# lhn0323/BEVFUSION-3D_object_detection

Hardware: AMD Instinct MI355X
Metric: nuScenes frames/sec (6-cam+LiDAR BEVFusion fwd+bwd) (higher is better)
Workload: dtype bf16; 1 GPU; full: BEVFusion camera+LiDAR (ResNet-50, LSS 6x256x704, hard voxelize 40k pts, sparse encoder, ConvFuser, SECOND/SECONDFPN, TransFusion head + Hungarian targets + focal/L1/gaussian-focal losses) fwd + bwd + clip + AdamW, bf16 autocast, fp32 index paths; global_batch=4, points_per_frame=40000, parallelism=independent frames per rank, execution=eager launches on 2 HIP queues (camera / BEV chain, LiDAR branch), view_transform_conv_dtype=bf16, head_fp32_conv=three bf16 products per multiply, fp32 accumulation (2^-16 relative per product), dense_weight_gradients=one grouped launch per tile shape at the end of the backward pass, backward_pass_thread=caller, trainable_params=37361053

## Files before the change

bevfusion-3d_object_detection_amd/_lib.py:

```python
import ctypes
import os

import torch

_HERE = os.path.dirname(os.path.abspath(__file__))
LIB_PATH = os.path.join(_HERE, "csrc", "libbevfusion_hip.so")

_c_int = ctypes.c_int
_c_vp = ctypes.c_void_p
_c_sz = ctypes.c_size_t

SIGNATURES = {
    "bfhip_abi_version": (_c_int, []),
    "bfhip_last_error": (ctypes.c_char_p, []),
    "bfhip_profile_enable": (None, [_c_int]),
    "bfhip_profile_read": (_c_int, [_c_int, _c_vp, _c_vp, _c_int]),
    "bfhip_bev_pool_fwd": (_c_int, [_c_vp] * 5 + [_c_int] * 7 + [_c_vp, _c_vp]),
    "bfhip_bev_pool_bwd": (_c_int, [_c_vp] * 5 + [_c_int] * 8 + [_c_vp, _c_vp]),
    "bfhip_dynamic_voxelize": (_c_int, [_c_vp, _c_vp, _c_int, _c_int, _c_vp, _c_vp, _c_vp]),
    "bfhip_hard_voxelize_workspace_bytes": (_c_sz, [_c_int, _c_int, _c_int]),
    "bfhip_hard_voxelize": (_c_int, [_c_vp, _c_int, _c_int, _c_vp, _c_vp, _c_vp, _c_vp, _c_vp,
                                     _c_int, _c_int, _c_vp, _c_sz, _c_vp, _c_vp]),
    "bfhip_bev_plan_workspace_bytes": (_c_sz, [ctypes.c_longlong, ctypes.c_longlong]),
    "bfhip_bev_plan": (_c_int, [_c_vp] * 7 + [_c_int] * 4 + [_c_vp] * 3 + [_c_vp] * 11 + [_c_int, _c_vp, _c_sz, _c_vp]),
# ... 93 lines not shown
                                     [_c_vp] * 4 + [_c_vp, _c_int, _c_vp, _c_vp, _c_vp]),
    "bfhip_bn2d_bwd_mask": (_c_int, [_c_vp] * 5 + [ctypes.c_longlong, _c_int, _c_int] + [_c_vp] * 4 + [_c_vp, _c_sz, _c_vp]),
    "bfhip_adamw_segment_bytes": (_c_int, []),
    "bfhip_adamw_chunk_elems": (_c_int, []),
    "bfhip_adamw_step": (_c_int, [_c_vp, _c_vp, _c_vp, _c_int, _c_vp, _c_vp] + [ctypes.c_float] * 6 + [_c_vp]),
    "bfhip_adamw_step_groups": (_c_int, [_c_vp, _c_vp, _c_vp, _c_int, _c_vp, _c_vp, _c_vp, _c_vp, _c_int, ctypes.c_float, _c_vp]),
    "bfhip_query_losses": (_c_int, [_c_vp] * 7 + [_c_int] * 6 + [ctypes.c_float, ctypes.c_float] + [_c_vp] * 4),
    "bfhip_swin_attn_supported": (_c_int, [_c_int] * 7),
    "bfhip_swin_attn_parts": (_c_int, [_c_int] * 4),
    "bfhip_swin_attn_fwd": (_c_int, [_c_vp, ctypes.c_longlong, _c_vp] + [_c_int] * 5 + [ctypes.c_float, _c_vp, _c_vp, _c_vp]),
    "bfhip_swin_attn_bwd": (_c_int, [_c_vp, ctypes.c_longlong, _c_vp, _c_vp, _c_vp, _c_vp] + [_c_int] * 5 +
                            [ctypes.c_float, _c_vp, _c_vp, _c_int, _c_vp]),
    "bfhip_layernorm_supported": (_c_int, [ctypes.c_longlong, _c_int, _c_int, _c_int]),
    "bfhip_layernorm_parts": (_c_int, [ctypes.c_longlong, _c_int]),
    "bfhip_layernorm_fwd": (_c_int, [_c_vp, _c_vp, _c_vp, ctypes.c_longlong, _c_vp, _c_vp, ctypes.c_longlong, _c_int, ctypes.c_float] +
                            [_c_int] * 3 + [_c_vp] * 4),
    "bfhip_layernorm_bwd": (_c_int, [_c_vp] * 6 + [ctypes.c_longlong, ctypes.c_longlong] + [_c_int] * 4 + [_c_vp] * 3 + [_c_int] +
                            [_c_vp] * 3),
    "bfhip_bn_eval_supported": (_c_int, [ctypes.c_longlong, _c_int, _c_int]),
    "bfhip_bn_eval_parts": (_c_int, [ctypes.c_longlong, _c_int, _c_int]),
    "bfhip_bn_eval_fwd": (_c_int, [_c_vp] * 6 + [ctypes.c_longlong, _c_int, _c_int, ctypes.c_float, _c_int, _c_vp, _c_vp]),
    "bfhip_bn_eval_bwd": (_c_int, [_c_vp] * 6 + [ctypes.c_longlong, _c_int, _c_int, ctypes.c_float, _c_int] + [_c_vp] * 5),
    "bfhip_img_preprocess_max_samples": (_c_int, []),
    "bfhip_img_preprocess": (_c_int, [_c_vp] + [_c_int] * 5 + [_c_vp, _c_vp, ctypes.c_float, _c_int, _c_int, _c_int, _c_int,
                                      _c_vp, _c_vp]),
    "bfhip_image_aug_max_taps": (_c_int, []),
    "bfhip_image_aug_max_cams": (_c_int, []),
    "bfhip_image_aug_supported": (_c_int, [_c_int] * 8),
    "bfhip_image_aug": (_c_int, [_c_vp, _c_int, _c_int, _c_vp, _c_vp, ctypes.c_longlong, _c_int, _c_int, _c_vp, _c_int, _c_int,
                                 _c_vp, _c_vp, ctypes.c_float] + [_c_int] * 4 + [_c_vp, _c_vp]),
    "bfhip_image_aug_masked": (_c_int, [_c_vp, _c_vp, _c_int, _c_int, _c_vp, _c_vp, ctypes.c_longlong, _c_int, _c_int, _c_vp, _c_int,
                                        _c_int, _c_vp, _c_vp, ctypes.c_float] + [_c_int] * 4 + [_c_vp, _c_vp]),
    "bfhip_points_aug_block": (_c_int, []),
    "bfhip_points_aug_workspace_bytes": (_c_sz, [ctypes.c_longlong, _c_int]),
    "bfhip_points_aug": (_c_int, [_c_vp, _c_int, _c_int, _c_vp, _c_vp, _c_vp, _c_sz, _c_vp]),
    "bfhip_points_aug_max_boxes": (_c_int, []),
    "bfhip_points_aug_paste": (_c_int, [_c_vp, _c_vp, _c_int, _c_int, _c_vp, _c_vp, _c_vp, _c_sz, _c_vp]),
    "bfhip_points_aug_max_sweeps": (_c_int, []),
    "bfhip_points_aug_sweeps": (_c_int, [_c_vp, _c_vp, _c_vp, _c_int, _c_int, _c_vp, _c_vp, _c_vp, _c_sz, _c_vp]),
    "bfhip_query_init_supported": (_c_int, [_c_int] * 8),
    "bfhip_query_init_workspace_bytes": (_c_sz, [_c_int] * 4),
    "bfhip_query_init_fwd": (_c_int, [_c_vp] + [ctypes.c_longlong] * 4 + [_c_int] * 4 + [ctypes.c_uint, _c_vp, ctypes.c_longlong,
                                      ctypes.c_longlong] + [_c_int] * 4 + [_c_vp] * 6 + [_c_sz, _c_vp]),
    "bfhip_query_init_bwd": (_c_int, [_c_vp, _c_vp, _c_int, _c_int, _c_int, ctypes.c_longlong, _c_int, _c_vp, _c_vp]),
    "bfhip_jpeg_parse": (_c_int, [_c_vp, _c_sz, _c_vp]),
    "bfhip_jpeg_entropy_decode": (_c_int, [_c_vp, _c_sz, _c_vp, _c_vp, _c_sz]),
    "bfhip_jpeg_decode": (_c_int, [_c_vp, _c_vp, _c_int, _c_vp, _c_sz, _c_vp, _c_sz, _c_vp, _c_sz, _c_vp]),
    "bfhip_points_in_boxes_block": (_c_int, []),
    "bfhip_points_in_boxes_max_boxes": (_c_int, []),
    "bfhip_points_in_boxes_workspace_bytes": (_c_sz, [ctypes.c_longlong, _c_int]),
    "bfhip_points_in_boxes_count": (_c_int, [_c_vp, ctypes.c_longlong, _c_int, _c_vp, _c_int, _c_vp, _c_vp, _c_vp, _c_sz, _c_vp]),
    "bfhip_points_in_boxes_gather": (_c_int, [_c_vp, ctypes.c_longlong, _c_int, _c_vp, _c_int, _c_vp, _c_vp, ctypes.c_longlong,
                                              _c_vp, ctypes.c_longlong, _c_vp, _c_sz, _c_vp]),
}


class ImgDesc(ctypes.Structure):
    _fields_ = [("data", _c_vp), ("h", _c_int), ("w", _c_int)]

_lib = None


def load():
    global _lib
    if _lib is None:
        if not os.path.exists(LIB_PATH):
            raise RuntimeError(
                "libbevfusion_hip.so not found at %s: build it with "
                "`python -c 'import __graft_entry__ as g; g.build()'` (hipcc, gfx950). "
                "There is no CPU fallback." % LIB_PATH)
        lib = ctypes.CDLL(LIB_PATH)
        for name, (res, args) in SIGNATURES.items():
            fn = getattr(lib, name)
            fn.restype = res
            fn.argtypes = args
        _lib = lib
    return _lib


_torch_ext = False


def torch_ext():
    global _torch_ext
    if _torch_ext is False:
        _torch_ext = None
        path = os.path.join(_HERE, "csrc", "bfhip_torch_ext.so")
        if os.environ.get("BFHIP_TORCH_EXT", "1") == "1" and os.path.exists(path):
            import importlib.util
            load()
            try:
                spec = importlib.util.spec_from_file_location("bfhip_torch_ext", path)
                mod = importlib.util.module_from_spec(spec)
                spec.loader.exec_module(mod)
                if mod.abi_version() == load().bfhip_abi_version():
                    _torch_ext = mod
            except (ImportError, OSError) as e:
                import warnings
                warnings.warn("bfhip_torch_ext not usable (%s); using the ctypes binding" % e)
    return _torch_ext


def check(rc, what):
    if rc != 0:
        msg = load().bfhip_last_error().decode("utf-8", "replace")
        raise RuntimeError("%s failed (rc=%d): %s" % (what, rc, msg))
# ... 64 lines not shown
```

bevfusion-3d_object_detection_amd/csrc/torch_binding.cpp:

```cpp
#include <torch/extension.h>
#include <torch/csrc/autograd/engine.h>
#include <torch/csrc/autograd/graph_task.h>
#include <c10/hip/HIPStream.h>
#include <c10/hip/HIPGuard.h>
#include <ATen/hip/impl/HIPStreamMasqueradingAsCUDA.h>
#include <hip/hip_runtime_api.h>

#include <map>
#include <mutex>
#include <vector>

#include "../../include/bevfusion_hip.h"

namespace {

using torch::Tensor;
using torch::autograd::AutogradContext;
using torch::autograd::tensor_list;

inline void *cur_stream(const Tensor &t) { return (void *)c10::hip::getCurrentHIPStream(t.get_device()).stream(); }
inline int dt_code(const Tensor &t) { return t.scalar_type() == at::kBFloat16 ? 1 : 0; }
inline void check(int rc, const char *what) {
  TORCH_CHECK(rc == 0, what, " failed (rc=", rc, "): ", bfhip_last_error());
}
// ... 403 lines not shown
    }
    dy = as_nhwc_bf16(dy);
    if (ctx->needs_input_grad(0)) {
      if (dgrad_lib) out[0] = add_grad(lib_dgrad(dy, x, weight, stride, pad, dil), d_alias, fork);
      else out[0] = hip_dgrad(dy, x, weight, wt, stride, pad, dil, d_alias, fork == 2 ? 2 : 1);
    }
    if (ctx->needs_input_grad(1)) out[1] = launch_wgrad(x, dy, weight, stride, pad, dil);
    if (has_bias && ctx->needs_input_grad(2)) out[2] = bias_grad(dy).to((at::ScalarType)g[6]);
    return out;
  }
};

tensor_list conv2d(const Tensor &x, const Tensor &weight, const c10::optional<Tensor> &bias, int64_t stride, int64_t pad, int64_t dil,
                   bool emit_stats, bool dgrad_lib, int64_t fork, const c10::optional<Tensor> &wt) {
  return ConvFn::apply(x, weight, bias, stride, pad, dil, emit_stats, dgrad_lib, fork, wt);
}

class LibConvFn : public torch::autograd::Function<LibConvFn> {
 public:
  static Tensor forward(AutogradContext *ctx, const Tensor &x_, const Tensor &weight, int64_t stride, int64_t pad, int64_t dil,
                        bool dgrad_hip, const c10::optional<Tensor> &wt) {
    Tensor x = as_nhwc_bf16(x_);
    Tensor w = weight.scalar_type() == at::kBFloat16 ? weight : weight.to(at::kBFloat16);
    Tensor y;
    {
      c10::impl::ExcludeDispatchKeyGuard no_autocast(c10::DispatchKey::AutocastCUDA);
      y = at::conv2d(x, w, {}, {stride, stride}, {pad, pad}, {dil, dil});
    }
    ctx->save_for_backward({x, weight, (wt.has_value() && wt->defined()) ? *wt : Tensor()});
    ctx->saved_data["geom"] = std::vector<int64_t>{stride, pad, dil, dgrad_hip ? 1 : 0};
    return y;
  }

  static tensor_list backward(AutogradContext *ctx, tensor_list grads) {
    auto saved = ctx->get_saved_variables();
    const Tensor &x = saved[0], &weight = saved[1], &wt = saved[2];
    const auto g = ctx->saved_data["geom"].toIntVector();
    const int64_t stride = g[0], pad = g[1], dil = g[2];
    tensor_list out(7);
    if (!grads[0].defined()) return out;
    Tensor dy = as_nhwc_bf16(grads[0]);
    if (ctx->needs_input_grad(0))
      out[0] = g[3] ? hip_dgrad(dy, x, weight, wt, stride, pad, dil, Tensor(), 1) : lib_dgrad(dy, x, weight, stride, pad, dil);
    if (ctx->needs_input_grad(1)) out[1] = launch_wgrad(x, dy, weight, stride, pad, dil);
    return out;
  }
};

Tensor lib_conv2d(const Tensor &x, const Tensor &weight, int64_t stride, int64_t pad, int64_t dil, bool dgrad_hip,
                  const c10::optional<Tensor> &wt) {
  return LibConvFn::apply(x, weight, stride, pad, dil, dgrad_hip, wt);
}

}

PYBIND11_MODULE(TORCH_EXTENSION_NAME, m) {
  m.doc() = "C++ autograd front-ends over libbevfusion_hip.so (include/bevfusion_hip.h)";
  m.def("bn2d", &bn2d, "fused BatchNorm2d(+residual)(+ReLU), channels-last, training mode; optional statistics partials of the producing conv",
        pybind11::arg("x"), pybind11::arg("residual"), pybind11::arg("weight"), pybind11::arg("bias"), pybind11::arg("running_mean"),
        pybind11::arg("running_var"), pybind11::arg("eps"), pybind11::arg("momentum"), pybind11::arg("relu"),
        pybind11::arg("partial") = c10::optional<Tensor>(), pybind11::arg("relu_bits") = false);
  m.def("bn1d", &bn1d, "fused BatchNorm1d(+residual)(+ReLU) on f32[N, C], training mode");
  m.def("conv2d", &conv2d, "dense convolution on csrc/conv2d.hip (conv2d.py::_Conv2dFunction): [y, partial (empty without statistics)[, x']]",
        pybind11::arg("x"), pybind11::arg("weight"), pybind11::arg("bias"), pybind11::arg("stride"), pybind11::arg("pad"), pybind11::arg("dil"),
        pybind11::arg("emit_stats"), pybind11::arg("dgrad_lib"), pybind11::arg("fork"), pybind11::arg("wt"));
  m.def("lib_conv2d", &lib_conv2d, "library forward, HIP weight gradient (conv2d.py::_LibConvHipWgradFunction)", pybind11::arg("x"),
        pybind11::arg("weight"), pybind11::arg("stride"), pybind11::arg("pad"), pybind11::arg("dil"), pybind11::arg("dgrad_hip"), pybind11::arg("wt"));
  m.def("defer_wgrad", &defer_wgrad, "queue a layer's weight gradient for the grouped launch at the end of the running backward pass");
  m.def("set_wgrad_grouped", [](bool on) { g_grouped = on; });
  m.def("pending_wgrads", &pending_wgrads);
  m.def("abi_version", []() { return bfhip_abi_version(); });
}
```

bevfusion-3d_object_detection_amd/depth_lss.py:

```python
import os
from typing import Tuple

import torch
from torch import nn

from . import _lib
from .bn2d import bn_act
from .conv2d import Conv2d
from .ops import bev_pool
from .registry import MODELS


BF16_BEV_OUT = os.environ.get("BFHIP_LIFT_SPLAT_BF16_OUT", "1") == "1"
CAMERA_MAJOR = os.environ.get("BFHIP_LIFT_SPLAT_ORDER", "0") == "1"
BF16_FEAT = os.environ.get("BFHIP_LIFT_SPLAT_BF16_FEAT", "1") == "1"


def _inverse(m):
    return torch.linalg.inv_ex(m, check_errors=False).inverse


def gen_dx_bx(xbound, ybound, zbound):
    rows = [xbound, ybound, zbound]
    dx = torch.Tensor([row[2] for row in rows])
    bx = torch.Tensor([row[0] + row[2] / 2.0 for row in rows])
    nx = torch.LongTensor([int((row[1] - row[0]) / row[2]) for row in rows])
    return dx, bx, nx


class BevPlan:

    def __init__(self, B, N, D, HW, nx, device, with_reference_outputs=False, with_geometry=False):
        self.B, self.N, self.D, self.HW = B, N, D, HW
        self.nx = [int(v) for v in nx]
        self.nprime = B * N * D * HW
        self.out_cells = B * self.nx[2] * self.nx[0] * self.nx[1]
        self.mmax = min(self.nprime, self.out_cells)
        i32 = dict(dtype=torch.int32, device=device)
        self.sorted_pd = torch.empty(self.nprime, **i32)
        self.starts = torch.empty(self.mmax, **i32)
        self.lengths = torch.empty(self.mmax, **i32)
        self.cell_of_interval = torch.empty(self.mmax, **i32)
        self.interval_order = torch.empty(self.mmax, **i32) if CAMERA_MAJOR else None
        self.counts = torch.zeros(2, **i32)
        self.cell_of_point = torch.empty(self.nprime, **i32)
        self.geom_sorted = torch.empty((self.nprime, 4), **i32) if with_reference_outputs else None
        self.ranks_sorted = torch.empty(self.nprime, dtype=torch.int64, device=device) if with_reference_outputs else None
        self.kept = torch.empty(self.nprime, dtype=torch.uint8, device=device) if with_reference_outputs else None
        self.geom_xyz = torch.empty((self.nprime, 3), dtype=torch.float32, device=device) if with_geometry else None
        nbytes = _lib.load().bfhip_bev_plan_workspace_bytes(self.nprime, self.out_cells)
        self.workspace = torch.empty(nbytes, dtype=torch.uint8, device=device)

    def build(self, frustum, post_trans, post_rots_inv, combine, c2l_trans, extra_rots, extra_trans, origin, dx):
        f32 = lambda t: t.contiguous().float()
        args = [f32(frustum), f32(post_trans), f32(post_rots_inv), f32(combine), f32(c2l_trans), f32(extra_rots),
                f32(extra_trans)]
        import ctypes
        nx_host = (ctypes.c_int32 * 3)(*self.nx)
        with torch.cuda.device(self.sorted_pd.device):
            rc = _lib.load().bfhip_bev_plan(
                *[_lib.ptr(a) for a in args], self.B, self.N, self.D, self.HW, _lib.host_f32(origin), _lib.host_f32(dx),
                nx_host, _lib.ptr(self.sorted_pd), _lib.ptr(self.starts), _lib.ptr(self.lengths),
                _lib.ptr(self.cell_of_interval), _lib.ptr(self.interval_order), _lib.ptr(self.counts), _lib.ptr(self.cell_of_point),
                _lib.ptr(self.geom_sorted), _lib.ptr(self.ranks_sorted), _lib.ptr(self.kept), _lib.ptr(self.geom_xyz),
                self.mmax, _lib.ptr(self.workspace), self.workspace.numel(), _lib.stream_of(self.sorted_pd))
        _lib.check(rc, "bev_plan")
        self._keepalive = args
        return self
# ... 7 lines not shown
        assert depth.dtype == torch.float32 and feat.dtype in (torch.float32, torch.bfloat16)
        f16 = 1 if feat.dtype == torch.bfloat16 else 0
        P, C = feat.shape
        assert P == plan.B * plan.N * plan.HW and depth.shape == (P, plan.D)
        assert out_dtype in (torch.float32, torch.bfloat16)
        out = torch.empty((plan.B, plan.nx[2], plan.nx[0], plan.nx[1], C), dtype=out_dtype, device=feat.device)
        with torch.cuda.device(feat.device):
            rc = _lib.load().bfhip_lift_splat_fwd(
                _lib.ptr(depth), depth.stride(0), _lib.ptr(feat), f16, feat.stride(0), _lib.ptr(plan.sorted_pd),
                _lib.ptr(plan.starts), _lib.ptr(plan.lengths), _lib.ptr(plan.cell_of_interval), _lib.ptr(plan.interval_order),
                _lib.ptr(plan.counts), plan.mmax, C, plan.out_cells, _lib.ptr(out), 1 if out_dtype == torch.bfloat16 else 0,
                _lib.stream_of(feat))
        _lib.check(rc, "lift_splat_fwd")
        ctx.save_for_backward(depth, feat)
        ctx.plan = plan
        return out

    @staticmethod
    def backward(ctx, out_grad):
        depth, feat = ctx.saved_tensors
        plan = ctx.plan
        out_grad = out_grad.contiguous()
        if out_grad.dtype not in (torch.float32, torch.bfloat16):
            out_grad = out_grad.float()
        P, C = feat.shape
        d_depth = torch.empty((P, plan.D), dtype=torch.float32, device=feat.device)
        d_feat = torch.empty((P, C), dtype=feat.dtype, device=feat.device)
        with torch.cuda.device(feat.device):
            rc = _lib.load().bfhip_lift_splat_bwd(
                _lib.ptr(out_grad), 1 if out_grad.dtype == torch.bfloat16 else 0, _lib.ptr(depth), depth.stride(0), _lib.ptr(feat),
                1 if feat.dtype == torch.bfloat16 else 0, feat.stride(0),
                _lib.ptr(plan.cell_of_point), plan.B * plan.N, plan.D, plan.HW, C, _lib.ptr(d_depth), plan.D,
                _lib.ptr(d_feat), C, _lib.stream_of(feat))
        _lib.check(rc, "lift_splat_bwd")
        return d_depth, d_feat, None, None


class _SplitDepthFeat(torch.autograd.Function):

    @staticmethod
    def forward(ctx, x, D, C):
        ctx.shape, ctx.D, ctx.C = x.shape, D, C
        return x[:, :D].float(), x[:, D:D + C].contiguous()

    @staticmethod
    def backward(ctx, g_logits, g_feat):
        D, C = ctx.D, ctx.C
        dx = torch.empty(ctx.shape, dtype=torch.bfloat16, device=g_logits.device)
        dx[:, :D].copy_(g_logits)
        dx[:, D:D + C].copy_(g_feat)
        if ctx.shape[1] > D + C:
            dx[:, D + C:].zero_()
        return dx, None, None


def lift_splat(depth, feat, plan, out_dtype=torch.float32):
    return _LiftSplat.apply(depth, feat, plan, out_dtype)


class BaseViewTransform(nn.Module):

    def __init__(self, in_channels: int, out_channels: int, image_size: Tuple[int, int],
                 feature_size: Tuple[int, int], xbound, ybound, zbound, dbound) -> None:
        super().__init__()
        self.in_channels = in_channels
        self.image_size = image_size
        self.feature_size = feature_size
        self.xbound, self.ybound, self.zbound, self.dbound = xbound, ybound, zbound, dbound
        dx, bx, nx = gen_dx_bx(xbound, ybound, zbound)
        self.dx = nn.Parameter(dx, requires_grad=False)
        self.bx = nn.Parameter(bx, requires_grad=False)
        self.nx = nn.Parameter(nx, requires_grad=False)
        self.C = out_channels
        self.conv_dtype = None
        self.frustum = self.create_frustum()
        self.D = self.frustum.shape[0]
        self.fp16_enabled = False
        self._nx_host = [int(v) for v in nx]
        self._dx_host = [float(v) for v in dx]
        self._origin_host = [float(v) for v in (bx - dx / 2.0)]

    def create_frustum(self):
        iH, iW = self.image_size
        fH, fW = self.feature_size
        ds = torch.arange(*self.dbound, dtype=torch.float).view(-1, 1, 1).expand(-1, fH, fW)
        D = ds.shape[0]
        xs = torch.linspace(0, iW - 1, fW, dtype=torch.float).view(1, 1, fW).expand(D, fH, fW)
        ys = torch.linspace(0, iH - 1, fH, dtype=torch.float).view(1, fH, 1).expand(D, fH, fW)
        return nn.Parameter(torch.stack((xs, ys, ds), -1), requires_grad=False)

    def make_plan(self, camera2lidar_rots, camera2lidar_trans, intrins_inverse, post_rots_inverse, post_trans,
                  extra_rots=None, extra_trans=None, with_reference_outputs=False, with_geometry=False):
        B, N, _ = camera2lidar_trans.shape
        dev = camera2lidar_trans.device
        fH, fW = self.feature_size
        plan = BevPlan(B, N, self.D, fH * fW, self._nx_host, dev, with_reference_outputs, with_geometry)
        combine = camera2lidar_rots.matmul(intrins_inverse)
        if extra_rots is None:
            extra_rots = torch.eye(3, device=dev).expand(B, 3, 3)
        if extra_trans is None:
            extra_trans = torch.zeros(B, 3, device=dev)
        return plan.build(self.frustum.reshape(-1, 3), post_trans.reshape(B * N, 3), post_rots_inverse.reshape(B * N, 9),
                          combine.reshape(B * N, 9), camera2lidar_trans.reshape(B * N, 3), extra_rots.reshape(B, 9),
                          extra_trans.reshape(B, 3), self._origin_host, self._dx_host)

    def get_geometry(self, camera2lidar_rots, camera2lidar_trans, intrins_inverse, post_rots_inverse, post_trans,
# ... 148 lines not shown
        return (depth, counts) if with_histogram else depth

    def depth_distribution(self, counts=None, depth=None):
        iH, iW = self.image_size
        fH, fW = self.feature_size
        if counts is None:
            BN = depth.shape[0]
            counts = torch.empty(BN, fH, fW, self.D, device=depth.device, dtype=torch.float32)
            depth = depth.contiguous().float()
        else:
            BN = counts.shape[0] * counts.shape[1]
        distr = torch.empty_like(counts)
        with torch.cuda.device(counts.device):
            rc = _lib.load().bfhip_depth_histogram(_lib.ptr(depth) if depth is not None else None, BN, iH, iW, fH, fW, self.D,
                                                   _lib.host_f32(self.dbound), _lib.ptr(counts), _lib.ptr(distr),
                                                   _lib.stream_of(counts))
        _lib.check(rc, "depth_histogram")
        return distr, counts

    def prepare(self, n_cams, points, lidar2image, cam_intrinsic, camera2lidar, img_aug_matrix, lidar_aug_matrix,
                lidar_aug_matrix_inverse=None, geom_feats_precomputed=None):
        depth_img, counts = self.rasterise_depth(n_cams, points, lidar2image, img_aug_matrix, lidar_aug_matrix,
                                                 lidar_aug_matrix_inverse, with_histogram=True)
        if isinstance(geom_feats_precomputed, BevPlan):
            plan = geom_feats_precomputed
        else:
            plan = self.make_plan(**self._calibration(cam_intrinsic, camera2lidar, img_aug_matrix, lidar_aug_matrix))
        prep = dict(depth_img=depth_img, counts=counts, plan=plan)
        prep.update(self.prepare_depth(depth_img, counts))
        return prep

    def prepare_depth(self, depth_img, counts):
        return {}

    @staticmethod
    def prepared_tensors(prep):
        out = [v for v in prep.values() if torch.is_tensor(v)]
        plan = prep.get("plan")
        if plan is not None:
            out += [v for v in vars(plan).values() if torch.is_tensor(v)]
        return out

    def forward(self, img, points, lidar2image, cam_intrinsic, camera2lidar, img_aug_matrix, lidar_aug_matrix,
                metas=None, camera_intrinsics_inverse=None, img_aug_matrix_inverse=None,
                lidar_aug_matrix_inverse=None, geom_feats_precomputed=None, prepared=None):
        if prepared is None:
            prepared = self.prepare(img.shape[1], points, lidar2image, cam_intrinsic, camera2lidar, img_aug_matrix,
                                    lidar_aug_matrix, lidar_aug_matrix_inverse, geom_feats_precomputed)
        depth_img, counts, plan = prepared["depth_img"], prepared["counts"], prepared["plan"]
        depth, feat, est_depth_distr, gt_depth_distr, counts_3d = self.get_depth_and_feat(img, depth_img, counts, prepared)
        x = self.lift_splat_bev(depth, feat, plan)
        if self.training:
            aux = getattr(self, "aux_stream", None)
            if aux is not None and est_depth_distr.is_cuda:
                aux.wait_stream(torch.cuda.current_stream(est_depth_distr.device))
                for t in (est_depth_distr, gt_depth_distr, counts_3d):
                    t.record_stream(aux)
                with torch.cuda.stream(aux):
                    depth_loss = self._depth_loss(est_depth_distr, gt_depth_distr, counts_3d)
            else:
                depth_loss = self._depth_loss(est_depth_distr, gt_depth_distr, counts_3d)
        else:
            depth_loss = 0.0
        return x, depth_loss

    def _depth_loss(self, est_depth_distr, gt_depth_distr, counts_3d):
        mask_flat = counts_3d.sum(dim=-1).view(-1) > 0
        gt = gt_depth_distr.view(-1, self.D)
        est = est_depth_distr.reshape(-1, self.D)
        cross_ent = -torch.sum(gt * torch.log(est + 1e-8), dim=-1)
        return torch.sum(cross_ent * mask_flat.float()) / (mask_flat.sum() + 1e-8)


class _DepthLift(torch.autograd.Function):

    @staticmethod
    def forward(ctx, d, weight, bias):
        y = torch.addcmul(bias.to(d.dtype), d, weight.reshape(1, 1, 1, -1).to(d.dtype))
        ctx.save_for_backward(d)
        ctx.dtypes = (weight.dtype, bias.dtype, weight.shape)
        return y

    @staticmethod
    def backward(ctx, dy):
        (d,) = ctx.saved_tensors
        wdt, bdt, wshape = ctx.dtypes
        if dy.dtype != torch.bfloat16 or not dy.is_contiguous() or dy.data_ptr() % 16:
            dy = dy.to(torch.bfloat16).contiguous()
        from . import _lib
        out = torch.empty(16, dtype=torch.float32, device=dy.device)
        ws = torch.empty(_lib.call_size("bfhip_depth_lift_bwd_workspace_bytes"), dtype=torch.uint8, device=dy.device)
        _lib.call("bfhip_depth_lift_bwd", dy.data_ptr(), d.data_ptr(), d.numel(), out.data_ptr(), ws.data_ptr(), ws.numel(),
                  _lib.stream_of(dy))
        return None, out[8:].to(wdt).reshape(wshape), out[:8].to(bdt)


@MODELS.register_module()
class DepthLSSTransform(BaseDepthTransform):

    def __init__(self, in_channels, out_channels, image_size, feature_size, xbound, ybound, zbound, dbound,
                 downsample: int = 1) -> None:
        super().__init__(in_channels, out_channels, image_size, feature_size, xbound, ybound, zbound, dbound)
        self.dtransform = nn.Sequential(
            nn.Conv2d(1, 8, 1), *bn_act(8),
            Conv2d(8, 32, 5, stride=4, padding=2), *bn_act(32),
            Conv2d(32, 64, 5, stride=2, padding=2), *bn_act(64))
        self.depthnet = nn.Sequential(
            Conv2d(in_channels + 64, in_channels, 3, padding=1), *bn_act(in_channels),
            Conv2d(in_channels, in_channels, 3, padding=1), *bn_act(in_channels),
            Conv2d(in_channels, self.D + self.C, 1))
        self.downsample = _make_downsample(out_channels, downsample)

    def run_dtransform(self, d):
        conv0 = self.dtransform[0]
        if not (d.is_cuda and d.dim() == 4 and d.shape[1] == 1 and conv0.kernel_size == (1, 1) and conv0.stride == (1, 1)):
            return self.dtransform(d)
        dt = torch.get_autocast_dtype("cuda") if torch.is_autocast_enabled("cuda") else d.dtype
        BN, _, H, W = d.shape
        if (dt == torch.bfloat16 and conv0.out_channels == 8 and conv0.bias is not None and torch.is_grad_enabled()
                and conv0.weight.requires_grad and not d.requires_grad):
            y = _DepthLift.apply(d.reshape(BN, H, W, 1).to(dt), conv0.weight, conv0.bias).permute(0, 3, 1, 2)
        else:
            w = conv0.weight.reshape(1, 1, 1, -1).to(dt)
            b = (conv0.bias if conv0.bias is not None else conv0.weight.new_zeros(w.shape[-1])).to(dt)
            y = torch.addcmul(b, d.reshape(BN, H, W, 1).to(dt), w).permute(0, 3, 1, 2)
        for layer in list(self.dtransform)[1:]:
            y = layer(y)
        return y

    def gt_depth_distribution(self, d, B, N):
        distr, counts = self.depth_distribution(depth=d)
        fH, fW = self.feature_size
        return distr.view(B, N, fH, fW, self.D), counts.view(B, N, fH, fW, self.D)

    def prepare_depth(self, depth_img, counts):
        B, N = depth_img.shape[:2]
        d = depth_img.reshape(B * N, *depth_img.shape[2:])
        if counts is not None:
            gt_depth_distr, counts_3d = self.depth_distribution(counts=counts)
        else:
            gt_depth_distr, counts_3d = self.gt_depth_distribution(d, B, N)
        with torch.autocast("cuda", dtype=self.conv_dtype or torch.bfloat16, enabled=self.conv_dtype is not None):
            dfeat = self.run_dtransform(d)
        return dict(gt_depth_distr=gt_depth_distr, counts_3d=counts_3d, dfeat=dfeat)

    def get_depth_and_feat(self, x, d, counts=None, prepared=None):
        B, N, C, fH, fW = x.shape
        BN = B * N
        x = x.reshape(BN, C, fH, fW)
        if prepared is None or "dfeat" not in prepared:
            prepared = self.prepare_depth(d, counts)
        gt_depth_distr, counts_3d, dfeat = prepared["gt_depth_distr"], prepared["counts_3d"], prepared["dfeat"]
        with torch.autocast("cuda", dtype=self.conv_dtype or torch.bfloat16, enabled=self.conv_dtype is not None):
            x = self.depthnet(torch.cat([dfeat, x], dim=1))
        if BF16_FEAT and x.dtype == torch.bfloat16 and x.is_cuda and self.C % 8 == 0:
            logits, feat_pm = _SplitDepthFeat.apply(x.permute(0, 2, 3, 1).reshape(BN * fH * fW, x.shape[1]), self.D, self.C)
            depth = logits.view(BN, fH, fW, self.D).softmax(dim=-1).permute(0, 3, 1, 2)
            feat = feat_pm.view(BN, fH, fW, self.C).permute(0, 3, 1, 2)
        else:
            x = x.float()
            depth = x[:, :self.D].softmax(dim=1)
            feat = x[:, self.D:self.D + self.C]
        est_depth_distr = depth.permute(0, 2, 3, 1).reshape(B, N, fH, fW, self.D)
        if self.training:
            depth_aux = gt_depth_distr.view(BN, fH, fW, self.D).permute(0, 3, 1, 2)
            depth = depth + (torch.maximum(depth_aux, depth) - depth).detach()
        return depth, feat, est_depth_distr, gt_depth_distr, counts_3d

    def get_cam_feats(self, x, d):
        B, N = x.shape[:2]
        depth, feat, est, gt, counts = self.get_depth_and_feat(x, d)
        fH, fW = depth.shape[-2:]
        out = depth.unsqueeze(1) * feat.unsqueeze(2)
        return out.reshape(B, N, self.C, self.D, fH, fW).permute(0, 1, 3, 4, 5, 2), est, gt, counts

    def forward(self, *args, **kwargs):
        x, depth_loss = super().forward(*args, **kwargs)
        with torch.autocast("cuda", dtype=self.conv_dtype or torch.bfloat16, enabled=self.conv_dtype is not None):
            x = self.downsample(x)
        return x, depth_loss
```

include/bevfusion_hip.h:

```cpp
#ifndef BEVFUSION_HIP_H_
#define BEVFUSION_HIP_H_

#include <stddef.h>
#include <stdint.h>

#ifdef __cplusplus
extern "C" {
#endif

#define BFHIP_OK 0
#define BFHIP_E_INVALID (-1)
#define BFHIP_E_WORKSPACE (-2)
#define BFHIP_E_LAUNCH (-3)

#define BFHIP_REDUCE_SUM 0
#define BFHIP_REDUCE_MEAN 1
#define BFHIP_REDUCE_MAX 2

#define BFHIP_OP_BEV_POOL_FWD 0
#define BFHIP_OP_BEV_POOL_BWD 1
#define BFHIP_OP_HARD_VOXELIZE 2
#define BFHIP_OP_DYNAMIC_VOXELIZE 3
#define BFHIP_OP_LIFT_SPLAT_FWD 4
#define BFHIP_OP_LIFT_SPLAT_BWD 5
// ... 375 lines not shown
int bfhip_query_init_fwd(const float *h, long long h_sb, long long h_sc, long long h_sy, long long h_sx, int B, int C, int H, int W,
                         unsigned nms_free_mask, const void *flat, long long flat_sb, long long flat_sr, int Ch, int row_dtype,
                         int K, int pos_w, long long *top_class, long long *top_index, float *query_pos,
                         float *query_heatmap_score, void *rows, void *workspace, size_t workspace_bytes, void *stream);
int bfhip_query_init_bwd(const long long *top_index, const void *d_rows, int B, int K, int Ch, long long HW, int row_dtype,
                         void *d_flat, void *stream);

#define BFHIP_JPEG_R_OK 0
#define BFHIP_JPEG_R_PROGRESSIVE 1
#define BFHIP_JPEG_R_ARITHMETIC 2
#define BFHIP_JPEG_R_PRECISION 3
#define BFHIP_JPEG_R_COMPONENTS 4
#define BFHIP_JPEG_R_MULTI_SCAN 5
#define BFHIP_JPEG_R_QUANT16 6
#define BFHIP_JPEG_R_SAMPLING 7
#define BFHIP_JPEG_R_EXIF_ORIENTATION 8
#define BFHIP_JPEG_R_NOT_BASELINE 9
#define BFHIP_JPEG_R_COLOUR_SPACE 10
typedef struct bfhip_jpeg_header {
  int32_t width, height, ncomp;
  int32_t supported, reason;
  int32_t restart_interval;
  int32_t mcus_x, mcus_y;
  int32_t hs[3], vs[3];
  int32_t block_cols[3], block_rows[3];
  int64_t coef_offset[3];
  int64_t coef_bytes;
  uint16_t quant[3][64];
} bfhip_jpeg_header;
typedef struct bfhip_jpeg_frame {
  int64_t coef_off[3];
  int64_t plane_off[3];
  int64_t rgb_off;
  int32_t width, height;
  int32_t hs, vs;
  int32_t block_cols[3], block_rows[3];
  uint16_t quant[3][64];
} bfhip_jpeg_frame;
int bfhip_jpeg_parse(const uint8_t *bytes, size_t n, bfhip_jpeg_header *header);
int bfhip_jpeg_entropy_decode(const uint8_t *bytes, size_t n, const bfhip_jpeg_header *header, int16_t *coef, size_t coef_bytes);
int bfhip_jpeg_decode(const bfhip_jpeg_frame *frames_host, const bfhip_jpeg_frame *frames_dev, int n_frames,
                      const int16_t *coef_dev, size_t coef_elems, uint8_t *planes_dev, size_t planes_bytes, uint8_t *rgb_dev,
                      size_t rgb_bytes, void *stream);

int bfhip_points_in_boxes_block(void);
int bfhip_points_in_boxes_max_boxes(void);
size_t bfhip_points_in_boxes_workspace_bytes(long long n, int K);
int bfhip_points_in_boxes_count(const float *points, long long n, int C, const float *planes, int K, int32_t *counts,
                                uint64_t *member, void *workspace, size_t workspace_bytes, void *stream);
int bfhip_points_in_boxes_gather(const float *points, long long n, int C, const float *centers, int K, const int32_t *counts,
                                 const uint64_t *member, long long total, float *out, long long capacity, const void *workspace,
                                 size_t workspace_bytes, void *stream);

#ifdef __cplusplus
}
#endif
#endif
```

Baseline: 157.5 frames/s.

## Fuse depth split, softmax, straight-through and depth cross-entropy into one kernel

```diff
diff --git a/bevfusion-3d_object_detection_amd/_lib.py b/bevfusion-3d_object_detection_amd/_lib.py
--- a/bevfusion-3d_object_detection_amd/_lib.py
+++ b/bevfusion-3d_object_detection_amd/_lib.py
@@ -169,6 +169,10 @@
     "bfhip_points_in_boxes_count": (_c_int, [_c_vp, ctypes.c_longlong, _c_int, _c_vp, _c_int, _c_vp, _c_vp, _c_vp, _c_sz, _c_vp]),
     "bfhip_points_in_boxes_gather": (_c_int, [_c_vp, ctypes.c_longlong, _c_int, _c_vp, _c_int, _c_vp, _c_vp, ctypes.c_longlong,
                                               _c_vp, ctypes.c_longlong, _c_vp, _c_sz, _c_vp]),
+    "bfhip_depth_tail_supported": (_c_int, [ctypes.c_longlong, _c_int, _c_int, _c_int]),
+    "bfhip_depth_tail_workspace_bytes": (_c_sz, [ctypes.c_longlong]),
+    "bfhip_depth_tail_fwd": (_c_int, [_c_vp, ctypes.c_longlong, _c_int, _c_int, _c_int] + [_c_vp] * 7 + [_c_vp, _c_sz, _c_vp]),
+    "bfhip_depth_tail_bwd": (_c_int, [_c_vp] * 7 + [ctypes.c_longlong, _c_int, _c_int, _c_int, _c_vp, _c_vp]),
 }
 
 
diff --git a/bevfusion-3d_object_detection_amd/csrc/depth_tail.hip b/bevfusion-3d_object_detection_amd/csrc/depth_tail.hip
--- /dev/null
+++ b/bevfusion-3d_object_detection_amd/csrc/depth_tail.hip
@@ -0,0 +1,245 @@
+#include "common.h"
+
+namespace bfhip {
+namespace {
+
+typedef unsigned short bf16_t;
+
+constexpr int kBlock = 256;
+constexpr int kWaves = kBlock / kWave;
+constexpr int kMaxSlots = 4;
+constexpr int kMaxBlocks = 2048;
+constexpr int kMaxLd = 8192;
+
+__device__ __forceinline__ unsigned rne(float f) {
+  unsigned u = __float_as_uint(f);
+  if ((u & 0x7fffffffu) > 0x7f800000u) return (u >> 16) | 0x40u;
+  return (u + 0x7fffu + ((u >> 16) & 1u)) >> 16;
+}
+
+__device__ __forceinline__ float wave_sum(float v) {
+#pragma unroll
+  for (int o = kWave / 2; o > 0; o >>= 1) v += __shfl_xor(v, o, kWave);
+  return v;
+}
+__device__ __forceinline__ float wave_max(float v) {
+#pragma unroll
+  for (int o = kWave / 2; o > 0; o >>= 1) v = fmaxf(v, __shfl_xor(v, o, kWave));
+  return v;
+}
+
+inline int grid_for(long long P) { return (int)(P < (long long)kMaxBlocks * kWaves ? (P + kWaves - 1) / kWaves : kMaxBlocks); }
+
+template <int NS, bool PAIR>
+__global__ __launch_bounds__(kBlock) void depth_tail_fwd_kernel(const bf16_t *__restrict__ x, long long P, int D, int C, int ldx,
+                                                                const float *__restrict__ gt, const float *__restrict__ counts,
+                                                                float *__restrict__ est, float *__restrict__ depth,
+                                                                bf16_t *__restrict__ feat, float *__restrict__ mask,
+                                                                double *__restrict__ partials) {
+  __shared__ double s_ce[kWaves], s_n[kWaves];
+  const int lane = threadIdx.x & (kWave - 1), wave = threadIdx.x / kWave;
+  double ce_acc = 0.0, n_acc = 0.0;
+  for (long long p = (long long)blockIdx.x * kWaves + wave; p < P; p += (long long)gridDim.x * kWaves) {
+    const bf16_t *xr = x + (size_t)p * ldx;
+    const size_t row = (size_t)p * D;
+    float v[NS], g[NS], cnt = 0.f;
+    float mx = -INFINITY;
+#pragma unroll
+    for (int k = 0; k < NS; ++k) {
+      const int d = lane + k * kWave;
+      const bool in = d < D;
+      v[k] = in ? __uint_as_float((unsigned)xr[d] << 16) : -INFINITY;
+      g[k] = in ? gt[row + d] : 0.f;
+      cnt += in ? counts[row + d] : 0.f;
+      mx = fmaxf(mx, v[k]);
+    }
+    if (PAIR) {
+      const unsigned *src = (const unsigned *)(xr + D);
+      unsigned *dst = (unsigned *)(feat + (size_t)p * C);
+      for (int c = lane; c < (C >> 1); c += kWave) dst[c] = src[c];
+    } else {
+      bf16_t *dst = feat + (size_t)p * C;
+      for (int c = lane; c < C; c += kWave) dst[c] = xr[D + c];
+    }
+    mx = wave_max(mx);
+    float sum = 0.f;
+#pragma unroll
+    for (int k = 0; k < NS; ++k) {
+      v[k] = (lane + k * kWave < D) ? expf(v[k] - mx) : 0.f;
+      sum += v[k];
+    }
+    sum = wave_sum(sum);
+    cnt = wave_sum(cnt);
+    float ce = 0.f;
+#pragma unroll
+    for (int k = 0; k < NS; ++k) {
+      const int d = lane + k * kWave;
+      if (d < D) {
+        const float e = v[k] / sum;
+        const float a = g[k];
+        const float m = (a != a) ? a : (a > e ? a : e);
+        est[row + d] = e;
+        depth[row + d] = e + (m - e);
+        ce += a * logf(e + 1e-8f);
+      }
+    }
+    ce = -wave_sum(ce);
+    const float mk = cnt > 0.f ? 1.f : 0.f;
+    if (lane == 0) mask[p] = mk;
+    ce_acc += (double)(ce * mk);
+    n_acc += (double)mk;
+  }
+  if (lane == 0) { s_ce[wave] = ce_acc; s_n[wave] = n_acc; }
+  __syncthreads();
+  if (threadIdx.x == 0) {
+    double a = 0.0, b = 0.0;
+#pragma unroll
+    for (int w = 0; w < kWaves; ++w) { a += s_ce[w]; b += s_n[w]; }
+    partials[2 * blockIdx.x] = a;
+    partials[2 * blockIdx.x + 1] = b;
+  }
+}
+
+__global__ __launch_bounds__(kBlock) void depth_tail_loss_kernel(const double *__restrict__ partials, int n, float *__restrict__ stats) {
+  __shared__ double s_a[kBlock], s_b[kBlock];
+  double a = 0.0, b = 0.0;
+  for (int i = threadIdx.x; i < n; i += kBlock) { a += partials[2 * i]; b += partials[2 * i + 1]; }
+  s_a[threadIdx.x] = a;
+  s_b[threadIdx.x] = b;
+  __syncthreads();
+  for (int o = kBlock / 2; o > 0; o >>= 1) {
+    if ((int)threadIdx.x < o) { s_a[threadIdx.x] += s_a[threadIdx.x + o]; s_b[threadIdx.x] += s_b[threadIdx.x + o]; }
+    __syncthreads();
+  }
+  if (threadIdx.x == 0) {
+    const float den = (float)s_b[0] + 1e-8f;
+    stats[0] = (float)s_a[0] / den;
+    stats[1] = den;
+  }
+}
+
+template <int NS, bool PAIR>
+__global__ __launch_bounds__(kBlock) void depth_tail_bwd_kernel(const float *__restrict__ d_depth, const bf16_t *__restrict__ d_feat,
+                                                                const float *__restrict__ est, const float *__restrict__ gt,
+                                                                const float *__restrict__ mask, const float *__restrict__ stats,
+                                                                const float *__restrict__ g_loss, long long P, int D, int C,
+                                                                int ldx, bf16_t *__restrict__ dx) {
+  const int lane = threadIdx.x & (kWave - 1), wave = threadIdx.x / kWave;
+  const float gl = g_loss ? g_loss[0] / stats[1] : 0.f;
+  for (long long p = (long long)blockIdx.x * kWaves + wave; p < P; p += (long long)gridDim.x * kWaves) {
+    const size_t row = (size_t)p * D;
+    bf16_t *out = dx + (size_t)p * ldx;
+    const float gce = -(gl * mask[p]);
+    float e[NS], g[NS], s = 0.f;
+#pragma unroll
+    for (int k = 0; k < NS; ++k) {
+      const int d = lane + k * kWave;
+      const bool in = d < D;
+      e[k] = in ? est[row + d] : 0.f;
+      const float a = in ? gt[row + d] : 0.f;
+      const float dd = in ? d_depth[row + d] : 0.f;
+      g[k] = in ? dd + (gce * a) / (e[k] + 1e-8f) : 0.f;
+      s += g[k] * e[k];
+    }
+    s = wave_sum(s);
+#pragma unroll
+    for (int k = 0; k < NS; ++k) {
+      const int d = lane + k * kWave;
+      if (d < D) out[d] = (bf16_t)rne((g[k] - s) * e[k]);
+    }
+    if (PAIR) {
+      const unsigned *src = (const unsigned *)(d_feat + (size_t)p * C);
+      unsigned *dst = (unsigned *)(out + D);
+      for (int c = lane; c < (C >> 1); c += kWave) dst[c] = src[c];
+    } else {
+      const bf16_t *src = d_feat + (size_t)p * C;
+      for (int c = lane; c < C; c += kWave) out[D + c] = src[c];
+    }
+    for (int c = D + C + lane; c < ldx; c += kWave) out[c] = 0;
+  }
+}
+
+bool supported(long long P, int D, int C, int ldx) {
+  return P >= 1 && P <= 0x7fffffffLL && D >= 1 && D <= kMaxSlots * kWave && C >= 8 && C % 8 == 0 && C <= kMaxLd &&
+         ldx >= D + C && ldx <= kMaxLd;
+}
+
+template <int NS>
+void launch_fwd(bool pair, int grid, hipStream_t s, const bf16_t *x, long long P, int D, int C, int ldx, const float *gt,
+                const float *counts, float *est, float *depth, bf16_t *feat, float *mask, double *partials) {
+  if (pair)
+    hipLaunchKernelGGL((depth_tail_fwd_kernel<NS, true>), dim3(grid), dim3(kBlock), 0, s, x, P, D, C, ldx, gt, counts, est, depth,
+                       feat, mask, partials);
+  else
+    hipLaunchKernelGGL((depth_tail_fwd_kernel<NS, false>), dim3(grid), dim3(kBlock), 0, s, x, P, D, C, ldx, gt, counts, est, depth,
+                       feat, mask, partials);
+}
+
+template <int NS>
+void launch_bwd(bool pair, int grid, hipStream_t s, const float *d_depth, const bf16_t *d_feat, const float *est, const float *gt,
+                const float *mask, const float *stats, const float *g_loss, long long P, int D, int C, int ldx, bf16_t *dx) {
+  if (pair)
+    hipLaunchKernelGGL((depth_tail_bwd_kernel<NS, true>), dim3(grid), dim3(kBlock), 0, s, d_depth, d_feat, est, gt, mask, stats,
+                       g_loss, P, D, C, ldx, dx);
+  else
+    hipLaunchKernelGGL((depth_tail_bwd_kernel<NS, false>), dim3(grid), dim3(kBlock), 0, s, d_depth, d_feat, est, gt, mask, stats,
+                       g_loss, P, D, C, ldx, dx);
+}
+
+}
+}
+
+using namespace bfhip;
+
+BFHIP_EXPORT int bfhip_depth_tail_supported(long long P, int D, int C, int ldx) { return supported(P, D, C, ldx) ? 1 : 0; }
+
+BFHIP_EXPORT size_t bfhip_depth_tail_workspace_bytes(long long P) {
+  if (P < 1) return 0;
+  return align_up((size_t)grid_for(P) * 2 * sizeof(double), 256);
+}
+
+BFHIP_EXPORT int bfhip_depth_tail_fwd(const void *x, long long P, int D, int C, int ldx, const float *gt, const float *counts,
+                                      float *est, float *depth, void *feat, float *mask, float *stats, void *workspace,
+                                      size_t workspace_bytes, void *stream) {
+  BFHIP_REQUIRE(supported(P, D, C, ldx), "depth_tail_fwd: unsupported shape P=%lld D=%d C=%d ldx=%d", P, D, C, ldx);
+  BFHIP_REQUIRE(x && gt && counts && est && depth && feat && mask && stats, "depth_tail_fwd: null pointer");
+  BFHIP_REQUIRE(((uintptr_t)x & 3) == 0 && ((uintptr_t)feat & 15) == 0, "depth_tail_fwd: x must be 4-byte and feat 16-byte aligned");
+  BFHIP_REQUIRE_WORKSPACE(workspace, workspace_bytes, bfhip_depth_tail_workspace_bytes(P), "depth_tail_fwd");
+  BFHIP_REQUIRE(((uintptr_t)workspace & 7) == 0, "depth_tail_fwd: workspace must be 8-byte aligned");
+  hipStream_t s = (hipStream_t)stream;
+  const int grid = grid_for(P);
+  const bool pair = (D % 2 == 0) && (ldx % 2 == 0);
+  double *partials = (double *)workspace;
+  const bf16_t *xp = (const bf16_t *)x;
+  bf16_t *fp = (bf16_t *)feat;
+  switch ((D + kWave - 1) / kWave) {
+    case 1: launch_fwd<1>(pair, grid, s, xp, P, D, C, ldx, gt, counts, est, depth, fp, mask, partials); break;
+    case 2: launch_fwd<2>(pair, grid, s, xp, P, D, C, ldx, gt, counts, est, depth, fp, mask, partials); break;
+    case 3: launch_fwd<3>(pair, grid, s, xp, P, D, C, ldx, gt, counts, est, depth, fp, mask, partials); break;
+    default: launch_fwd<4>(pair, grid, s, xp, P, D, C, ldx, gt, counts, est, depth, fp, mask, partials); break;
+  }
+  int rc = check_launch("depth_tail_fwd");
+  if (rc != BFHIP_OK) return rc;
+  hipLaunchKernelGGL(depth_tail_loss_kernel, dim3(1), dim3(kBlock), 0, s, (const double *)partials, grid, stats);
+  return check_launch("depth_tail_loss");
+}
+
+BFHIP_EXPORT int bfhip_depth_tail_bwd(const float *d_depth, const void *d_feat, const float *est, const float *gt, const float *mask,
+                                      const float *stats, const float *g_loss, long long P, int D, int C, int ldx, void *dx,
+                                      void *stream) {
+  BFHIP_REQUIRE(supported(P, D, C, ldx), "depth_tail_bwd: unsupported shape P=%lld D=%d C=%d ldx=%d", P, D, C, ldx);
+  BFHIP_REQUIRE(d_depth && d_feat && est && gt && mask && stats && dx, "depth_tail_bwd: null pointer");
+  BFHIP_REQUIRE(((uintptr_t)dx & 3) == 0 && ((uintptr_t)d_feat & 3) == 0, "depth_tail_bwd: dx and d_feat must be 4-byte aligned");
+  hipStream_t s = (hipStream_t)stream;
+  const int grid = grid_for(P);
+  const bool pair = (D % 2 == 0) && (ldx % 2 == 0);
+  const bf16_t *df = (const bf16_t *)d_feat;
+  bf16_t *dxp = (bf16_t *)dx;
+  switch ((D + kWave - 1) / kWave) {
+    case 1: launch_bwd<1>(pair, grid, s, d_depth, df, est, gt, mask, stats, g_loss, P, D, C, ldx, dxp); break;
+    case 2: launch_bwd<2>(pair, grid, s, d_depth, df, est, gt, mask, stats, g_loss, P, D, C, ldx, dxp); break;
+    case 3: launch_bwd<3>(pair, grid, s, d_depth, df, est, gt, mask, stats, g_loss, P, D, C, ldx, dxp); break;
+    default: launch_bwd<4>(pair, grid, s, d_depth, df, est, gt, mask, stats, g_loss, P, D, C, ldx, dxp); break;
+  }
+  return check_launch("depth_tail_bwd");
+}
diff --git a/bevfusion-3d_object_detection_amd/csrc/torch_binding.cpp b/bevfusion-3d_object_detection_amd/csrc/torch_binding.cpp
--- a/bevfusion-3d_object_detection_amd/csrc/torch_binding.cpp
+++ b/bevfusion-3d_object_detection_amd/csrc/torch_binding.cpp
@@ -479,6 +479,53 @@
   return LibConvFn::apply(x, weight, stride, pad, dil, dgrad_hip, wt);
 }
 
+class DepthTailFn : public torch::autograd::Function<DepthTailFn> {
+ public:
+  static tensor_list forward(AutogradContext *ctx, const Tensor &x, const Tensor &gt, const Tensor &counts, int64_t D, int64_t C) {
+    ctx->set_materialize_grads(false);
+    const int64_t P = x.size(0), ldx = x.size(1);
+    const auto f32 = x.options().dtype(at::kFloat);
+    Tensor est = at::empty({P, D}, f32), depth = at::empty({P, D}, f32);
+    Tensor feat = at::empty({P, C}, x.options());
+    Tensor mask = at::empty({P}, f32), stats = at::empty({2}, f32);
+    const size_t wsb = bfhip_depth_tail_workspace_bytes(P);
+    Tensor ws = at::empty({(int64_t)wsb}, x.options().dtype(at::kByte));
+    check(bfhip_depth_tail_fwd(x.data_ptr(), P, (int)D, (int)C, (int)ldx, gt.data_ptr<float>(), counts.data_ptr<float>(),
+                               est.data_ptr<float>(), depth.data_ptr<float>(), feat.data_ptr(), mask.data_ptr<float>(),
+                               stats.data_ptr<float>(), ws.data_ptr(), wsb, cur_stream(x)),
+          "depth_tail_fwd");
+    ctx->save_for_backward({est, gt, mask, stats});
+    ctx->saved_data["dims"] = std::vector<int64_t>{P, D, C, ldx};
+    ctx->mark_non_differentiable({est});
+    return {depth, feat, est, stats.select(0, 0)};
+  }
+
+  static tensor_list backward(AutogradContext *ctx, tensor_list grads) {
+    auto saved = ctx->get_saved_variables();
+    const Tensor &est = saved[0], &gt = saved[1], &mask = saved[2], &stats = saved[3];
+    const auto dims = ctx->saved_data["dims"].toIntVector();
+    const int64_t P = dims[0], D = dims[1], C = dims[2], ldx = dims[3];
+    Tensor d_depth = grads[0].defined() ? grads[0] : at::zeros_like(est);
+    Tensor d_feat = grads[1].defined() ? grads[1] : at::zeros({P, C}, est.options().dtype(at::kBFloat16));
+    if (d_depth.scalar_type() != at::kFloat) d_depth = d_depth.to(at::kFloat);
+    if (d_feat.scalar_type() != at::kBFloat16) d_feat = d_feat.to(at::kBFloat16);
+    d_depth = d_depth.contiguous();
+    d_feat = d_feat.contiguous();
+    Tensor g_loss = grads[3];
+    if (g_loss.defined()) g_loss = (g_loss.scalar_type() == at::kFloat ? g_loss : g_loss.to(at::kFloat)).contiguous();
+    Tensor dx = at::empty({P, ldx}, est.options().dtype(at::kBFloat16));
+    check(bfhip_depth_tail_bwd(d_depth.data_ptr<float>(), d_feat.data_ptr(), est.data_ptr<float>(), gt.data_ptr<float>(),
+                               mask.data_ptr<float>(), stats.data_ptr<float>(), g_loss.defined() ? g_loss.data_ptr<float>() : nullptr,
+                               P, (int)D, (int)C, (int)ldx, dx.data_ptr(), cur_stream(est)),
+          "depth_tail_bwd");
+    return {dx, Tensor(), Tensor(), Tensor(), Tensor()};
+  }
+};
+
+tensor_list depth_tail(const Tensor &x, const Tensor &gt, const Tensor &counts, int64_t D, int64_t C) {
+  return DepthTailFn::apply(x, gt, counts, D, C);
+}
+
 }
 
 PYBIND11_MODULE(TORCH_EXTENSION_NAME, m) {
@@ -496,5 +543,7 @@
   m.def("defer_wgrad", &defer_wgrad, "queue a layer's weight gradient for the grouped launch at the end of the running backward pass");
   m.def("set_wgrad_grouped", [](bool on) { g_grouped = on; });
   m.def("pending_wgrads", &pending_wgrads);
+  m.def("depth_tail", &depth_tail, "split + softmax + straight-through depth + depth cross-entropy behind the depthnet, training "
+        "(depth_lss.py::_DepthTail): [depth, feat, est, loss]");
   m.def("abi_version", []() { return bfhip_abi_version(); });
 }
diff --git a/bevfusion-3d_object_detection_amd/depth_lss.py b/bevfusion-3d_object_detection_amd/depth_lss.py
--- a/bevfusion-3d_object_detection_amd/depth_lss.py
+++ b/bevfusion-3d_object_detection_amd/depth_lss.py
@@ -14,6 +14,7 @@
 BF16_BEV_OUT = os.environ.get("BFHIP_LIFT_SPLAT_BF16_OUT", "1") == "1"
 CAMERA_MAJOR = os.environ.get("BFHIP_LIFT_SPLAT_ORDER", "0") == "1"
 BF16_FEAT = os.environ.get("BFHIP_LIFT_SPLAT_BF16_FEAT", "1") == "1"
+DEPTH_TAIL = os.environ.get("BFHIP_DEPTH_TAIL", "1") == "1"
 
 
 def _inverse(m):
@@ -127,6 +128,64 @@
         if ctx.shape[1] > D + C:
             dx[:, D + C:].zero_()
         return dx, None, None
+
+
+class _DepthTail(torch.autograd.Function):
+
+    @staticmethod
+    def forward(ctx, x, gt, counts, D, C):
+        P, ldx = x.shape
+        dev = x.device
+        f32 = dict(dtype=torch.float32, device=dev)
+        est, depth = torch.empty((P, D), **f32), torch.empty((P, D), **f32)
+        feat = torch.empty((P, C), dtype=torch.bfloat16, device=dev)
+        mask, stats = torch.empty(P, **f32), torch.empty(2, **f32)
+        ws = torch.empty(_lib.call_size("bfhip_depth_tail_workspace_bytes", P), dtype=torch.uint8, device=dev)
+        with torch.cuda.device(dev):
+            _lib.call("bfhip_depth_tail_fwd", x.data_ptr(), P, D, C, ldx, gt.data_ptr(), counts.data_ptr(), est.data_ptr(),
+                      depth.data_ptr(), feat.data_ptr(), mask.data_ptr(), stats.data_ptr(), ws.data_ptr(), ws.numel(),
+                      _lib.stream_of(x))
+        ctx.save_for_backward(est, gt, mask, stats)
+        ctx.dims = (P, D, C, ldx)
+        ctx.mark_non_differentiable(est)
+        ctx.set_materialize_grads(False)
+        return depth, feat, est, stats[0]
+
+    @staticmethod
+    def backward(ctx, d_depth, d_feat, _d_est, g_loss):
+        est, gt, mask, stats = ctx.saved_tensors
+        P, D, C, ldx = ctx.dims
+        if d_depth is None:
+            d_depth = torch.zeros_like(est)
+        if d_feat is None:
+            d_feat = torch.zeros((P, C), dtype=torch.bfloat16, device=est.device)
+        d_depth = d_depth.contiguous() if d_depth.dtype == torch.float32 else d_depth.float().contiguous()
+        d_feat = d_feat.contiguous() if d_feat.dtype == torch.bfloat16 else d_feat.to(torch.bfloat16).contiguous()
+        if g_loss is not None:
+            g_loss = g_loss.contiguous() if g_loss.dtype == torch.float32 else g_loss.float().contiguous()
+        dx = torch.empty((P, ldx), dtype=torch.bfloat16, device=est.device)
+        with torch.cuda.device(est.device):
+            _lib.call("bfhip_depth_tail_bwd", d_depth.data_ptr(), d_feat.data_ptr(), est.data_ptr(), gt.data_ptr(), mask.data_ptr(),
+                      stats.data_ptr(), _lib.ptr(g_loss), P, D, C, ldx, dx.data_ptr(), _lib.stream_of(est))
+        return dx, None, None, None, None
+
+
+def depth_tail(x_pm, gt, counts, D, C):
+    ext = _lib.torch_ext()
+    if ext is not None and hasattr(ext, "depth_tail"):
+        with torch.cuda.device(x_pm.device):
+            return ext.depth_tail(x_pm, gt, counts, D, C)
+    return _DepthTail.apply(x_pm, gt, counts, D, C)
+
+
+def depth_tail_supported(x_pm, gt, counts, D, C):
+    if not (DEPTH_TAIL and x_pm.is_cuda and x_pm.dtype == torch.bfloat16 and x_pm.dim() == 2 and x_pm.is_contiguous()):
+        return False
+    P = x_pm.shape[0]
+    for t in (gt, counts):
+        if not (t.is_cuda and t.dtype == torch.float32 and t.is_contiguous() and t.numel() == P * D):
+            return False
+    return _lib.load().bfhip_depth_tail_supported(P, D, C, x_pm.shape[1]) == 1
 
 
 def lift_splat(depth, feat, plan, out_dtype=torch.float32):
@@ -381,7 +440,10 @@
         x = self.lift_splat_bev(depth, feat, plan)
         if self.training:
             aux = getattr(self, "aux_stream", None)
-            if aux is not None and est_depth_distr.is_cuda:
+            fused = getattr(self, "_fused_depth_loss", None)
+            if fused is not None:
+                depth_loss, self._fused_depth_loss = fused, None
+            elif aux is not None and est_depth_distr.is_cuda:
                 aux.wait_stream(torch.cuda.current_stream(est_depth_distr.device))
                 for t in (est_depth_distr, gt_depth_distr, counts_3d):
                     t.record_stream(aux)
@@ -473,7 +535,7 @@
             dfeat = self.run_dtransform(d)
         return dict(gt_depth_distr=gt_depth_distr, counts_3d=counts_3d, dfeat=dfeat)
 
-    def get_depth_and_feat(self, x, d, counts=None, prepared=None):
+    def get_depth_and_feat(self, x, d, counts=None, prepared=None, fuse_loss=True):
         B, N, C, fH, fW = x.shape
         BN = B * N
         x = x.reshape(BN, C, fH, fW)
@@ -482,6 +544,17 @@
         gt_depth_distr, counts_3d, dfeat = prepared["gt_depth_distr"], prepared["counts_3d"], prepared["dfeat"]
         with torch.autocast("cuda", dtype=self.conv_dtype or torch.bfloat16, enabled=self.conv_dtype is not None):
             x = self.depthnet(torch.cat([dfeat, x], dim=1))
+        self._fused_depth_loss = None
+        x_pm = None
+        if fuse_loss and self.training and BF16_FEAT and DEPTH_TAIL and x.dtype == torch.bfloat16 and x.is_cuda:
+            x_pm = x.permute(0, 2, 3, 1).reshape(BN * fH * fW, x.shape[1])
+            if not depth_tail_supported(x_pm, gt_depth_distr, counts_3d, self.D, self.C):
+                x_pm = None
+        if x_pm is not None:
+            depth_pm, feat_pm, est_pm, self._fused_depth_loss = depth_tail(x_pm, gt_depth_distr, counts_3d, self.D, self.C)
+            depth = depth_pm.view(BN, fH, fW, self.D).permute(0, 3, 1, 2)
+            feat = feat_pm.view(BN, fH, fW, self.C).permute(0, 3, 1, 2)
+            return depth, feat, est_pm.view(B, N, fH, fW, self.D), gt_depth_distr, counts_3d
         if BF16_FEAT and x.dtype == torch.bfloat16 and x.is_cuda and self.C % 8 == 0:
             logits, feat_pm = _SplitDepthFeat.apply(x.permute(0, 2, 3, 1).reshape(BN * fH * fW, x.shape[1]), self.D, self.C)
             depth = logits.view(BN, fH, fW, self.D).softmax(dim=-1).permute(0, 3, 1, 2)
@@ -498,7 +571,7 @@
 
     def get_cam_feats(self, x, d):
         B, N = x.shape[:2]
-        depth, feat, est, gt, counts = self.get_depth_and_feat(x, d)
+        depth, feat, est, gt, counts = self.get_depth_and_feat(x, d, fuse_loss=False)
         fH, fW = depth.shape[-2:]
         out = depth.unsqueeze(1) * feat.unsqueeze(2)
         return out.reshape(B, N, self.C, self.D, fH, fW).permute(0, 1, 3, 4, 5, 2), est, gt, counts
diff --git a/include/bevfusion_hip.h b/include/bevfusion_hip.h
--- a/include/bevfusion_hip.h
+++ b/include/bevfusion_hip.h
@@ -451,6 +451,14 @@
                                  const uint64_t *member, long long total, float *out, long long capacity, const void *workspace,
                                  size_t workspace_bytes, void *stream);
 
+int bfhip_depth_tail_supported(long long P, int D, int C, int ldx);
+size_t bfhip_depth_tail_workspace_bytes(long long P);
+int bfhip_depth_tail_fwd(const void *x, long long P, int D, int C, int ldx, const float *gt, const float *counts, float *est,
+                         float *depth, void *feat, float *mask, float *stats, void *workspace, size_t workspace_bytes,
+                         void *stream);
+int bfhip_depth_tail_bwd(const float *d_depth, const void *d_feat, const float *est, const float *gt, const float *mask,
+                         const float *stats, const float *g_loss, long long P, int D, int C, int ldx, void *dx, void *stream);
+
 #ifdef __cplusplus
 }
 #endif
```

After: 151.0 frames/s. -4.2%, worse.
